# vinhisreal/YOLO-LitePi

Measured on AMD Instinct MI355X. Metric: images/sec end-to-end (det+NMS+clf) 640x640 batch64, higher is better.
Workload: dtype f16; 1 GPU; configs[2]: full det+NMS+ROI+ShuffleNetV2 pipeline, fp16, batch=64/GPU, 640x640, inputs resident in HBM; classifier=ShuffleNetV2 x1.0, 91 classes, seeded random weights, 64x64 ROIs, min_area=50, max_det=300, steps_in_flight=3, distinct_input_batches=4, global_batch=64, boxes_pre_area_filter_rank0=413

## Files before the change

yolo-litepi_amd/csrc/conv_kernels.hip:

```cpp
#include "common.h"
#include "conv.h"
#include "conv_bounds.h"
#include <type_traits>
#include <algorithm>
#include <utility>

namespace lp {

typedef _Float16 half_t;
typedef _Float16 half8 __attribute__((ext_vector_type(8)));
typedef _Float16 half4 __attribute__((ext_vector_type(4)));
typedef _Float16 half2v __attribute__((ext_vector_type(2)));
typedef float floatx4 __attribute__((ext_vector_type(4)));
typedef float floatx2 __attribute__((ext_vector_type(2)));
typedef uint32_t u32x4 __attribute__((ext_vector_type(4)));

enum { EPI_PLAIN = 0, EPI_SHUFFLE = 1 };

#define LP_STAMP(k)                                                                                   \
  if (a.stamps && threadIdx.x == 0)                                                                   \
    a.stamps[((size_t)(blockIdx.z * gridDim.y + blockIdx.y) * gridDim.x + blockIdx.x) * 16 + (k)] = \
        (k) == 0 ? wall_clock64() : clock64();

template <typename T> struct Tr;
// ... 435 lines not shown
  }
  LP_STAMP(10)

  const int oy = oy0 + ly;
  const int oxb = ox0 + wx * 20 + (col & 3);
  if constexpr (T2 > 0) {
    typename Tr<T>::frag w2f[T2][TailSteps<T>::per_nt(NT)];
    floatx4 bias2[T2];
    tail_load<T, NT, T2>(a, lane, g, w2f, bias2);
    ConvArgs a2 = a;
    a2.Cout = a.Cout2; a2.act = a.act2; a2.res = nullptr;
#pragma unroll
    for (int p = 0; p < 5; ++p) {
      const int ox = oxb + p * 4;
      if (oy < a.Hout && ox < a.Wout) {
        const long pix = (n * a.Hout + oy) * a.Wout + ox;
        floatx4 v[NT];
#pragma unroll
        for (int t = 0; t < NT; ++t) v[t] = acc[t][p];
        if (a.act == ACT_SILU) tail_store<T, NT, T2, ACT_SILU>(a2, pix, g, v, bias_r, w2f, bias2);
        else tail_store<T, NT, T2, ACT_NONE>(a2, pix, g, v, bias_r, w2f, bias2);
      }
    }
  } else {
    if (a.act == ACT_SILU) epilogue_tile<T, NT, ACT_SILU>(a, acc, bias_r, n, ns, g, oy, oxb);
    else if (a.act == ACT_RELU) epilogue_tile<T, NT, ACT_RELU>(a, acc, bias_r, n, ns, g, oy, oxb);
    else epilogue_tile<T, NT, ACT_NONE>(a, acc, bias_r, n, ns, g, oy, oxb);
  }
  LP_STAMP(11)
  if (a.stamps && threadIdx.x == 0) a.stamps[((size_t)(blockIdx.z * gridDim.y + blockIdx.y) * gridDim.x + blockIdx.x) * 16 + 12] = wall_clock64();
}


#define BN_STAMP(k)                                                                                                   \
  if (a.stamps && threadIdx.x == 0)                                                                                 \
    a.stamps[((size_t)blockIdx.y * gridDim.x + blockIdx.x) * 16 + (k)] = ((k) == 0 || (k) == 15) ? wall_clock64() : clock64();
template <typename T, int NT, int P1, int P2, bool SEP, int T2 = 0, int SG = 0, bool CL = false>
__global__ __launch_bounds__(256, ((NT >= 4 || P1 >= 15 || (NT == 2 && P1 == 5)) ? 2 : 3)) void bottleneck_mfma_kernel(const BneckArgs a) {
  static_assert(!CL || (SEP && T2 > 0 && SG > 0), "CL: the staged tile must survive conv_a, and cv2's gather must be the straight-line form");
  extern __shared__ __attribute__((aligned(16))) char smem[];
  constexpr int G = Tr<T>::G;
  const int tid = threadIdx.x, lane = tid & 63, wave = tid >> 6;
  const int g = lane >> 4, col = lane & 15;
  const int tile_id = a.tile_major ? blockIdx.x : blockIdx.y;
  const int ty = (int)((tile_id * a.rcp_tx) >> 16), tx = tile_id - ty * a.tiles_x;
  const int n = a.tile_major ? blockIdx.y : blockIdx.x;
  BN_STAMP(0)
  BN_STAMP(1)
  const int TH = a.TH, TW = a.TW, LW = a.LW, PS = a.PS, S = a.steps, CG = a.CG;
  const int PSA = CL ? a.PSA : PS;
  const int CGA = CL ? a.kg : CG;
  const int c1off = CL ? (a.kg - CG) * 16 : 0;
  const int oy0 = ty * TH, ox0 = tx * TW;
  const int IH = TH + 4, IW = TW + 4, H1 = TH + 2, W1 = TW + 2;
  const int R1 = H1 * W1, R2 = TH * TW;
  const int n1 = (R1 + 15) >> 4, n2 = (R2 + 15) >> 4;

  int* lds_toff = reinterpret_cast<int*>(smem);
  const int wbytes = S * NT * 1024;
  const u32x4* lds_w1 = reinterpret_cast<const u32x4*>(smem + 512);
  const u32x4* lds_w2 = reinterpret_cast<const u32x4*>(smem + 512 + wbytes);
  constexpr int SR = TailSteps<T>::per_nt(NT);
  const int w3frags = T2 > 0 ? T2 * (a.sg + SR) : 0;
  const u32x4* lds_w3 = reinterpret_cast<const u32x4*>(smem + 512 + 2 * wbytes);
  char* tile = smem + 512 + 2 * wbytes + w3frags * 1024;
  char* tile2 = SEP ? tile + (TH + 4) * LW * PSA : tile;
  for (int q = tid; q < S * 4; q += 256) {
    int tap = (int)(((unsigned)q * a.rcp_cg) >> 16);
    const int cg = q - tap * CG;
    tap = tap > 8 ? 8 : tap;
    const int ky = (tap * 21846) >> 16, kx = tap - 3 * ky;
    lds_toff[q] = (ky * LW + kx) * PSA + c1off + cg * 16;
    if (CL) lds_toff[64 + q] = (ky * LW + kx) * PS + cg * 16;
  }

  const int RS = LW * (PSA >> 4), PSs = PSA >> 4;
  const int pcs = (RS + 63) >> 6;
  constexpr int NPC = CL ? 4 : 3;
  const int st_pitch = CL ? a.cat_pitch : a.in_pitch;
  const int iy0 = oy0 - 2, ix0 = ox0 - 2;
  const char* zeros = reinterpret_cast<const char*>(a.zeros);
  {
    const int wave_s = __builtin_amdgcn_readfirstlane(wave);
    for (int p = wave_s; p < 2 * S * NT; p += 4) {
      const u32x4* src = p < S * NT ? reinterpret_cast<const u32x4*>(a.w1) + p * 64 : reinterpret_cast<const u32x4*>(a.w2) + (p - S * NT) * 64;
      LP_GLDS16(src + lane, smem + 512 + p * 1024);
    }
    for (int p = wave_s; p < w3frags; p += 4) LP_GLDS16(reinterpret_cast<const u32x4*>(a.w3) + p * 64 + lane, smem + 512 + 2 * wbytes + p * 1024);
    const char* in_b = reinterpret_cast<const char*>(CL ? a.cat : a.in);
// ... 14 lines not shown
        const bool rok = gy >= 0 && gy < a.H;
        const char* rowp = in_b + ((long)(n * a.H + (rok ? gy : 0)) * a.W + ix0) * st_pitch * (long)sizeof(T);
#pragma unroll
        for (int pc = 0; pc < NPC; ++pc) {
          if (pc < pcs) {
            const char* src = (rok && lok[pc]) ? rowp + voff[pc] : zeros;
            if (inrs[pc]) LP_GLDS16(src, tile + (iy * RS + pc * 64) * 16);
          }
        }
      }
    } else {
      const int nitems = IH * pcs;
      for (int it = wave_s; it < nitems; it += 4) {
        const int iy = (int)(((unsigned)it * a.rcp_pcs) >> 16), pc = it - iy * pcs;
        const int gy = iy0 + iy;
        const char* rowp = in_b + ((long)(n * a.H + gy) * a.W + ix0) * st_pitch * (long)sizeof(T);
        const int sl = pc * 64 + lane;
        const int ix = (int)(((unsigned)sl * a.rcp_ps) >> 16), cgs = sl - ix * PSs;
        const int gx = ix0 + ix;
        const bool ok = gy >= 0 && gy < a.H && gx >= 0 && gx < a.W && ix < IW && cgs < CGA;
        const char* src = ok ? rowp + (ix * st_pitch + cgs * G) * (int)sizeof(T) : zeros;
        if (sl < RS) LP_GLDS16(src, tile + (iy * RS + pc * 64) * 16);
      }
    }
  }
  BN_STAMP(2)
  floatx4 bias1[NT], bias2[NT];
#pragma unroll
  for (int t = 0; t < NT; ++t) {
    bias1[t] = *reinterpret_cast<const floatx4*>(a.b1 + g * 4 * NT + t * 4);
    bias2[t] = *reinterpret_cast<const floatx4*>(a.b2 + g * 4 * NT + t * 4);
  }

  int pk1[P1], pb1[P1];
#pragma unroll
  for (int i = 0; i < P1; ++i) {
    int p = (wave + 4 * i) * 16 + col;
    p = p < R1 ? p : R1 - 1;
    const int py = (int)(((unsigned)p * a.rcp_w1) >> 16), px = p - py * W1;
    pk1[i] = (py << 16) | px;
    pb1[i] = (py * LW + px) * PSA;
  }
  floatx4 acc[NT][P1];
#pragma unroll
  for (int t = 0; t < NT; ++t)
#pragma unroll
    for (int i = 0; i < P1; ++i) acc[t][i] = floatx4{0.f, 0.f, 0.f, 0.f};
  asm volatile("s_waitcnt vmcnt(0) lgkmcnt(0)" ::: "memory");
  __builtin_amdgcn_s_barrier();
  BN_STAMP(3)
  for (int s = 0; s < S; ++s) {
    const int toff = lds_toff[4 * s + g];
    typename Tr<T>::frag af[NT], bf[P1];
#pragma unroll
    for (int t = 0; t < NT; ++t) af[t] = as_frag<T>(lds_w1[(s * NT + t) * 64 + lane]);
#pragma unroll
    for (int i = 0; i < P1; ++i) bf[i] = as_frag<T>(*reinterpret_cast<const u32x4*>(tile + pb1[i] + toff));
#pragma unroll
    for (int t = 0; t < NT; ++t)
#pragma unroll
      for (int i = 0; i < P1; ++i) acc[t][i] = Tr<T>::mma(af[t], bf[i], acc[t][i]);
  }
  BN_STAMP(4)
  if (!SEP) {
    asm volatile("s_waitcnt lgkmcnt(0)" ::: "memory");
    __builtin_amdgcn_s_barrier();
  }
  auto write_mid = [&](auto interior_tag) {
    constexpr bool INTERIOR = decltype(interior_tag)::value;
#pragma unroll
    for (int i = 0; i < P1; ++i) {
      const int p = (wave + 4 * i) * 16 + col;
      if (wave + 4 * i < n1 && p < R1) {
        const int py = pk1[i] >> 16, px = pk1[i] & 0xffff;
        bool inside = true;
        if constexpr (!INTERIOR) {
          const int gy = oy0 - 1 + py, gx = ox0 - 1 + px;
          inside = gy >= 0 && gy < a.H && gx >= 0 && gx < a.W;
        }
        T* dst = reinterpret_cast<T*>(tile2 + (py * LW + px) * PS) + g * 4 * NT;
#pragma unroll
        for (int t = 0; t < NT; ++t) {
          if (g * 4 * NT + t * 4 < a.C) {
            typename Tr<T>::quad q;
            const floatx4 y = act4<T, ACT_SILU>(acc[t][i], bias1[t]);
#pragma unroll
            for (int r = 0; r < 4; ++r) q[r] = inside ? (T)y[r] : (T)0.f;
            *reinterpret_cast<typename Tr<T>::quad*>(dst + t * 4) = q;
          }
        }
      }
    }
  };
  if (oy0 >= 1 && ox0 >= 1 && oy0 + TH + 1 <= a.H && ox0 + TW + 1 <= a.W) write_mid(std::true_type{});
  else write_mid(std::false_type{});
  asm volatile("s_waitcnt lgkmcnt(0)" ::: "memory");
  __builtin_amdgcn_s_barrier();

  BN_STAMP(5)
  int pk2[P2], pb2[P2];
#pragma unroll
  for (int i = 0; i < P2; ++i) {
    int p = (wave + 4 * i) * 16 + col;
    p = p < R2 ? p : R2 - 1;
    const int oy = (int)(((unsigned)p * a.rcp_tw) >> 16), ox = p - oy * TW;
    pk2[i] = (oy << 16) | ox;
    pb2[i] = (oy * LW + ox) * PS;
  }
  floatx4 acc2[NT][P2];
#pragma unroll
  for (int t = 0; t < NT; ++t)
#pragma unroll
    for (int i = 0; i < P2; ++i) acc2[t][i] = floatx4{0.f, 0.f, 0.f, 0.f};
  for (int s = 0; s < S; ++s) {
    const int toff = lds_toff[(CL ? 64 : 0) + 4 * s + g];
    typename Tr<T>::frag af[NT], bf[P2];
#pragma unroll
    for (int t = 0; t < NT; ++t) af[t] = as_frag<T>(lds_w2[(s * NT + t) * 64 + lane]);
#pragma unroll
    for (int i = 0; i < P2; ++i) bf[i] = as_frag<T>(*reinterpret_cast<const u32x4*>(tile2 + pb2[i] + toff));
#pragma unroll
    for (int t = 0; t < NT; ++t)
#pragma unroll
      for (int i = 0; i < P2; ++i) acc2[t][i] = Tr<T>::mma(af[t], bf[i], acc2[t][i]);
  }
  BN_STAMP(6)
  const int chbase = g * 4 * NT;
  if constexpr (T2 == 0) {
#pragma unroll
    for (int i = 0; i < P2; ++i) {
      const int p = (wave + 4 * i) * 16 + col;
      const int gy = oy0 + (pk2[i] >> 16), gx = ox0 + (pk2[i] & 0xffff);
      if (wave + 4 * i < n2 && p < R2 && gy < a.H && gx < a.W) {
        const int pix = (n * a.H + gy) * a.W + gx;
        floatx4 v[NT];
#pragma unroll
        for (int t = 0; t < NT; ++t) v[t] = acc2[t][i];
        const T* xres = SEP ? reinterpret_cast<const T*>(tile + (((pk2[i] >> 16) + 2) * LW + (pk2[i] & 0xffff) + 2) * PSA + c1off) + chbase
                            : reinterpret_cast<const T*>(a.in) + eoff(pix, a.in_pitch) + chbase;
        store_lane_at<T, NT, ACT_SILU>(reinterpret_cast<T*>(a.out) + eoff(pix, a.out_pitch) + chbase, xres, chbase, a.C, v, bias2);
      }
    }
  } else {
    constexpr int SGMAX = sizeof(T) == 2 ? 3 : 6;
    const int sg_n = SG > 0 ? SG : a.sg;
    const int ST = sg_n + SR;
    floatx4 bias3[T2];
#pragma unroll
    for (int t = 0; t < T2; ++t) bias3[t] = *reinterpret_cast<const floatx4*>(a.b3 + g * 4 * T2 + t * 4);
    constexpr int LA = P2 < 4 ? P2 : 4;
    auto tile_pixel = [&](int i, bool& valid) {
      const int p = (wave + 4 * i) * 16 + col;
      const int gy = oy0 + (pk2[i] >> 16), gx = ox0 + (pk2[i] & 0xffff);
      valid = wave + 4 * i < n2 && p < R2 && gy < a.H && gx < a.W;
      return valid ? (n * a.H + gy) * a.W + gx : 0;
    };
    constexpr bool FLAT = SG > 0;
    constexpr int SGN = FLAT ? SG : SGMAX;
    typename Tr<T>::quad xq[LA][NT];
    auto request = [&](int i, u32x4 (&dst)[SGN], typename Tr<T>::quad (&xdst)[NT]) {
      bool valid;
      const int pix = tile_pixel(i, valid);
      if (FLAT && !SEP) {
        const T* xp = reinterpret_cast<const T*>(a.in) + eoff(pix, a.in_pitch);
#pragma unroll
        for (int t = 0; t < NT; ++t) xdst[t] = *reinterpret_cast<const typename Tr<T>::quad*>(xp + (chbase + t * 4 < a.C ? chbase + t * 4 : 0));
      }
      const T* catpix = reinterpret_cast<const T*>(a.cat) + eoff(pix, a.cat_pitch);
      const char* ldspix = tile + (((pk2[i] >> 16) + 2) * LW + (pk2[i] & 0xffff) + 2) * PSA;
#pragma unroll
      for (int s = 0; s < SGN; ++s) {
        const int grp = 4 * s + g;
        if constexpr (CL) {
          dst[s] = *reinterpret_cast<const u32x4*>(ldspix + (grp < a.kg ? grp * 16 : 0));
        } else if (FLAT) {
          dst[s] = *reinterpret_cast<const u32x4*>(catpix + (grp < a.kg ? grp * G : 0));
        } else {
          dst[s] = u32x4{0u, 0u, 0u, 0u};
          if (s < a.sg && valid && grp < a.kg) dst[s] = *reinterpret_cast<const u32x4*>(catpix + grp * G);
        }
      }
    };
    u32x4 bgq[LA][SGN];
#pragma unroll
    for (int i = 0; i < LA; ++i) request(i, bgq[i], xq[i]);
    __builtin_amdgcn_sched_barrier(0);
#pragma unroll
    for (int i = 0; i < P2; ++i) {
      if (!FLAT && wave + 4 * i >= n2) continue;
      bool valid;
      const int pix = tile_pixel(i, valid);
      typename Tr<T>::frag bg[SGN];
#pragma unroll
      for (int s = 0; s < SGN; ++s) {
        const unsigned m = (!FLAT || (valid && 4 * s + g < a.kg)) ? 0xffffffffu : 0u;
        bg[s] = as_frag<T>(bgq[i % LA][s] & m);
      }
      typename Tr<T>::quad xqi[NT];
#pragma unroll
      for (int t = 0; t < NT; ++t) xqi[t] = xq[i % LA][t];
      if (i + LA < P2) {
        request(i + LA, bgq[i % LA], xq[i % LA]);
        __builtin_amdgcn_sched_barrier(0);
      }
      const T* xres = SEP ? reinterpret_cast<const T*>(tile + (((pk2[i] >> 16) + 2) * LW + (pk2[i] & 0xffff) + 2) * PSA + c1off) + chbase
                          : reinterpret_cast<const T*>(a.in) + eoff(pix, a.in_pitch) + chbase;
      T yl[NT][4];
#pragma unroll
      for (int t = 0; t < NT; ++t) {
        typename Tr<T>::quad xr;
#pragma unroll
        for (int r = 0; r < 4; ++r) xr[r] = (T)0.f;
        if (SEP) {
          if (chbase + t * 4 < a.C) xr = *reinterpret_cast<const typename Tr<T>::quad*>(xres + t * 4);
        } else if (FLAT) {
          if (valid && chbase + t * 4 < a.C) xr = xqi[t];
        } else if (valid && chbase + t * 4 < a.C) xr = *reinterpret_cast<const typename Tr<T>::quad*>(xres + t * 4);
        const floatx4 y = act4<T, ACT_SILU>(acc2[t][i], bias2[t]);
#pragma unroll
        for (int r = 0; r < 4; ++r) {
          const T q = (T)y[r];
          yl[t][r] = (T)((float)q + (float)xr[r]);
        }
      }
      typename Tr<T>::frag bq[SR];
      if constexpr (sizeof(T) == 2) {
#pragma unroll
        for (int s = 0; s < SR; ++s)
#pragma unroll
          for (int r = 0; r < 4; ++r) {
            bq[s][r] = yl[2 * s][r];
            bq[s][4 + r] = (2 * s + 1 < NT) ? yl[(2 * s + 1 < NT) ? 2 * s + 1 : 0][r] : (T)0.f;
          }
      } else {
#pragma unroll
        for (int s = 0; s < SR; ++s)
#pragma unroll
          for (int r = 0; r < 4; ++r) bq[s][r] = yl[s][r];
      }
      floatx4 o[T2];
#pragma unroll
      for (int t = 0; t < T2; ++t) o[t] = floatx4{0.f, 0.f, 0.f, 0.f};
#pragma unroll
      for (int s = 0; s < SGN; ++s) {
        if (FLAT || s < a.sg) {
#pragma unroll
          for (int t = 0; t < T2; ++t) o[t] = Tr<T>::mma(as_frag<T>(lds_w3[(t * ST + s) * 64 + lane]), bg[s], o[t]);
        }
      }
#pragma unroll
      for (int s = 0; s < SR; ++s)
#pragma unroll
        for (int t = 0; t < T2; ++t) o[t] = Tr<T>::mma(as_frag<T>(lds_w3[(t * ST + sg_n + s) * 64 + lane]), bq[s], o[t]);
      if (valid) {
        T* o3 = reinterpret_cast<T*>(a.out3) + eoff(pix, a.out3_pitch) + g * 4 * T2;
        if (a.act3 == ACT_SILU) store_lane_at<T, T2, ACT_SILU>(o3, nullptr, g * 4 * T2, a.C3, o, bias3);
        else store_lane_at<T, T2, ACT_NONE>(o3, nullptr, g * 4 * T2, a.C3, o, bias3);
      }
    }
  }
  BN_STAMP(7)
  BN_STAMP(15)
}

template <typename T, int NT, int NP, int EPI, bool UPS = false>
__global__ __launch_bounds__(256) void conv1x1_mfma_kernel(const ConvArgs a) {
  extern __shared__ __attribute__((aligned(16))) char smem[];
  constexpr int G = Tr<T>::G;
  const int tid = threadIdx.x;
  const int lane = tid & 63, wave = tid >> 6;
  const int g = lane >> 4, col = lane & 15;
  const int ns = blockIdx.y;
  const int S = a.steps;
  const int CG = a.Cin / G;

  const long M = a.m_dyn ? (long)(*a.m_dyn) * a.pix_per_item : (long)a.M;
  const long ntiles = (M + 64 * NP - 1) / (64 * NP);
  if ((long)blockIdx.x >= ntiles) return;

  u32x4* lds_w = reinterpret_cast<u32x4*>(smem);
  const u32x4* wsrc = reinterpret_cast<const u32x4*>(a.wpk) + (size_t)ns * S * NT * 64;
  for (int i = tid; i < S * NT * 64; i += 256) lds_w[i] = wsrc[i];
  __syncthreads();
  const T* in = reinterpret_cast<const T*>(a.in);
  floatx4 bias_r[NT];
#pragma unroll
  for (int t = 0; t < NT; ++t) bias_r[t] = *reinterpret_cast<const floatx4*>(a.bias + ns * 16 * NT + g * 4 * NT + t * 4);

  for (long tile = blockIdx.x; tile < ntiles; tile += gridDim.x) {
    const long pix0 = (tile * 4 + wave) * 16 * NP;
    if (pix0 >= M) continue;
    const T* src[NP];
// ... 1006 lines not shown
template <typename T> static bool launch_bneck(const BottleneckPair& bp, const BneckArgs& a, dim3 grid, hipStream_t st) {
  return for_each_entry(cplan::kBneckTiles, [&](auto i) {
    constexpr int TILE = (int)decltype(i)::value;
    constexpr cplan::BneckTile t = cplan::kBneckTiles[TILE];
    if (bp.TH != t.th || bp.TW != t.tw) return false;
    if (bp.T2 == 0)
      return for_each_entry(cplan::kBneckNT, [&](auto n) {
        constexpr int nt = cplan::kBneckNT[decltype(n)::value];
        if constexpr (nt <= t.max_nt) {
          if (bp.NT != nt) return false;
          launch_bneck_kernel<T, nt, t.p1, t.p2, 0, 0, false>(a, grid, bp.lds_bytes, st);
          return true;
        } else {
          return false;
        }
      });
    if constexpr (sizeof(T) == 2) {
      static_assert(cplan::kBneckMaxSgF16 == 3, "one launch_bneck_tail line per SG");
      switch (bp.sg) {
        case 1: return launch_bneck_tail<T, TILE, 1>(bp, a, grid, st);
        case 2: return launch_bneck_tail<T, TILE, 2>(bp, a, grid, st);
        case 3: return launch_bneck_tail<T, TILE, 3>(bp, a, grid, st);
        default: return false;
      }
    } else {
      return bp.sg <= cplan::kBneckMaxSgF32 && launch_bneck_tail<T, TILE, 0>(bp, a, grid, st);
    }
  });
}

void BottleneckPair::launch(const View& in, const View& out, int N, hipStream_t st, const View* cat) const {
  LP_CHECK(in.C == C && in.H == out.H && in.W == out.W, LP_ERR_STATE, "bottleneck: view mismatch");
  LP_CHECK((in.pitch % 8) == 0 && (out.pitch % 4) == 0, LP_ERR_STATE, "unaligned channel pitch");
  LP_CHECK(span_ok(N, in) && span_ok(N, out) && (!cat || span_ok(N, *cat)), LP_ERR_ARG, "bottleneck: a tensor of batch %d exceeds 2^31 elements", N);
  BneckArgs k;
  memset(&k, 0, sizeof(k));
  k.in = in.base; k.out = out.base; k.w1 = a.d_w.p; k.w2 = b.d_w.p; k.b1 = a.d_bias.as<float>(); k.b2 = b.d_bias.as<float>();
  k.zeros = a.d_bias.as<float>() + round_up(C, 64);
  k.N = N; k.H = in.H; k.W = in.W; k.C = C; k.in_pitch = in.pitch; k.out_pitch = out.pitch;
  k.TH = TH; k.TW = TW; k.tiles_x = ceil_div(in.W, TW); k.LW = LW; k.PS = PS; k.CG = CG; k.steps = steps;
  if (T2) {
    LP_CHECK(cat && cat->base && cat->H == in.H && cat->W == in.W && out.C >= C3, LP_ERR_STATE, "bottleneck+cv2: concat view missing or output too narrow");
    k.w3 = d_w3.p; k.b3 = d_b3.as<float>(); k.cat = cat->base; k.cat_pitch = cat->pitch;
    k.out3 = out.base; k.out3_pitch = out.pitch; k.C3 = C3; k.act3 = act3; k.kg = kg; k.sg = sg;
    k.out = nullptr;
    if (cl) {
      const size_t es = prec == LP_FP16 ? 2 : 4;
      LP_CHECK(reinterpret_cast<const char*>(in.base) == reinterpret_cast<const char*>(cat->base) + (size_t)(kg * cplan::group(prec) - C) * es &&
                   in.pitch == cat->pitch,
               LP_ERR_STATE, "bottleneck %s: planned with the input as the concat's last stored segment, launched with another view", name.c_str());
      k.PSA = PSA;
    }
  } else {
    LP_CHECK(out.C >= C, LP_ERR_STATE, "bottleneck: output view too narrow");
  }
  const int tiles_y = ceil_div(in.H, TH);
  k.rcp_tx = rcp16_checked(k.tiles_x, k.tiles_x * tiles_y);
  k.rcp_cg = rcp_cg; k.rcp_ps = rcp_ps; k.rcp_pcs = rcp_pcs; k.rcp_w1 = rcp_w1; k.rcp_tw = rcp_tw;
  k.tile_major = tile_major_order();
  dim3 grid(N, k.tiles_x * tiles_y);
  if (k.tile_major) grid = dim3(k.tiles_x * tiles_y, N);
  static const char* stamp_path = getenv("LITEPI_BNECK_STAMPS");
  DevBuf d_stamps;
  if (stamp_path && *stamp_path) {
    d_stamps.alloc((size_t)grid.x * grid.y * 16 * 8);
    LP_HIP(hipMemsetAsync(d_stamps.p, 0, (size_t)grid.x * grid.y * 16 * 8, st));
    k.stamps = d_stamps.as<unsigned long long>();
// ... 144 lines not shown
```

yolo-litepi_amd/csrc/conv_plan.h:

```cpp
#pragma once
#include <cstddef>

#include "../../include/litepi.h"

namespace lp {
namespace cplan {

constexpr int cdiv(int a, int b) { return (a + b - 1) / b; }
inline int group(int prec) { return prec == LP_FP16 ? 8 : 4; }

inline unsigned rcp16(int d, int range) {
  const unsigned m = (65536u + d - 1) / d;
  for (int x = 0; x < range; ++x)
    if ((int)((x * m) >> 16) != x / d) return 0;
  return m;
}

struct Variant { int nt, t2; };
constexpr Variant kConv3x3[] = {{1, 0}, {2, 0}, {3, 0}, {4, 0}, {4, 4}, {2, 1}};
constexpr Variant kConvS2[] = {{1, 0}, {2, 0}, {3, 0}, {4, 0}, {1, 1}, {2, 2}, {4, 4}};
constexpr int s2_unroll(int steps) { return steps >= 5 ? 4 : 1; }
constexpr int kConv1x1[] = {1, 2, 3, 4};
constexpr int kStemCO[] = {8, 16, 32};
struct BneckTile { int th, tw, p1, p2, max_nt; bool tail, cl; };
// ... 123 lines not shown
    p.CK = cin;
    p.CGc = cin / G;
    p.nchunks = 1;
    p.steps = cdiv(p.CGc, 4);
    while (p.NT > 1 && (size_t)p.steps * p.NT * 1024 > 96 * 1024) --p.NT;
    p.nsplits = cdiv(tiles_total, p.NT);
    p.lds_bytes = (size_t)p.steps * p.NT * 1024;
    if (p.lds_bytes > 160 * 1024) p.plan_err = "conv1x1 weights do not fit LDS";
  }
  return p;
}

inline bool conv_tail_supported(int k, int stride, int cmid, int cout2) {
  if (k != 3 || cmid % 8 != 0) return false;
  const int nt = cdiv(cmid, 16), t2 = cdiv(cout2, 16);
  return t2 > 0 && (stride == 1 ? has_variant(kConv3x3, nt, t2) : stride == 2 ? has_variant(kConvS2, nt, t2) : false);
}
inline int tail_steps(int prec, int nt) { return prec == LP_FP16 ? (nt + 1) / 2 : nt; }

struct BneckTail {
  int cat_global = 0, c3 = 0;
  bool in_is_last_stored = false;
  bool cl = false;
};
struct BneckTiling {
  bool ok = false;
  int TH = 8, TW = 40, LW = 0;
  size_t lds_bytes = 0;
  int T2 = 0, kg = 0, sg = 0;
  bool cl = false;
  int PSA = 0;
};

inline BneckTiling plan_bneck(int prec, int c, int h, int w, int batch_hint, const BneckTail* tail) {
  BneckTiling p;
  const int G = group(prec);
  if (c % 8 != 0 || c > 64) return p;
  const int nt = cdiv(c, 16), cg = c / G;
  size_t extra_lds = 0;
  if (tail) {
    if (tail->cat_global <= 0 || tail->cat_global % G != 0 || tail->c3 % 8 != 0) return p;
    p.T2 = cdiv(tail->c3, 16);
    p.kg = tail->cat_global / G;
    p.sg = cdiv(p.kg, 4);
    if (!has_variant(kBneckTails, nt, p.T2) || p.sg > (prec == LP_FP16 ? kBneckMaxSgF16 : kBneckMaxSgF32)) return p;
    extra_lds = (size_t)p.T2 * (p.sg + tail_steps(prec, nt)) * 1024;
  }
  const int steps = cdiv(9 * cg, 4);
  if (steps * 4 > 128) return p;
  const int pss = lds_pixel_slots(cg);
  const int B = batch_hint > 0 ? batch_hint : 1;
  const bool sep = nt == 1;
  const int kg_cl = (tail && tail->in_is_last_stored) ? p.kg : 0;
  const bool try_cl = tail && tail->cl && kg_cl > cg && kg_cl <= 4 && prec == LP_FP16 && nt == 1;
  for (int pass = try_cl ? 0 : 1; pass < 2; ++pass) {
    const bool clp = pass == 0;
    const int pssa = clp ? (kg_cl | 1) : pss;
    long best = -1;
    for (const BneckTile& t : kBneckTiles) {
      const int TH = t.th, TW = t.tw;
      if (nt > t.max_nt || (tail && !t.tail) || (clp && !t.cl)) continue;
      if ((TH == 20 || TH == 10) && (long)cdiv(h, TH) * cdiv(w, TW) * B > 512) continue;
      int l = TW + 4;
      if (cg <= 1) while (l % 16 != 2) ++l;
      if (cdiv(l * pssa, 64) > (clp ? 4 : 8)) continue;
      const size_t need = 512 + (size_t)2 * steps * nt * 1024 + extra_lds + (size_t)(TH + 4) * l * pssa * 16 + (size_t)(sep ? TH + 2 : 0) * l * pss * 16;
// ... 21 lines not shown
```

yolo-litepi_amd/csrc/detector_plan.cpp:

```cpp
#include "detector.h"
#include <cstring>

#include <algorithm>
#include <optional>
#include <set>

namespace lp {

struct PlanSwitches {
  static bool on(const char* name) { return getenv(name) != nullptr; }
  bool no_c2f = on("LITEPI_NO_C2F");
  bool c2f_bb80 = on("LITEPI_C2F_BB80");
  std::string c2f_skip = getenv("LITEPI_C2F_SKIP") ? std::string(";") + getenv("LITEPI_C2F_SKIP") + ";" : std::string();
  int c2f_min_batch = getenv("LITEPI_C2F_MIN_BATCH") ? atoi(getenv("LITEPI_C2F_MIN_BATCH")) : 4;
  bool c2f_store_all = on("LITEPI_C2F_STORE_ALL");
  bool c2f_xcv1 = on("LITEPI_C2F_XCV1");
  bool no_c2f_xcv1 = on("LITEPI_NO_C2F_XCV1");
  bool no_s2c = on("LITEPI_NO_S2C");
  bool no_s2lds = on("LITEPI_NO_S2LDS");
  bool no_s2tail = on("LITEPI_NO_S2TAIL");
  bool no_sppf_fused = on("LITEPI_NO_SPPF_FUSED");
  bool no_sibling = on("LITEPI_NO_SIBLING");
  bool no_bneck = on("LITEPI_NO_BNECK");
  bool no_cv2fuse = on("LITEPI_NO_CV2FUSE");
// ... 826 lines not shown
  tensors_.push_back(M);
  op.in = tin; op.out = (int)tensors_.size() - 1;
  ops_.push_back(op);
  done[sib] = 1;
  return true;
}

bool Planner::try_bottleneck(const ConvSite& c) {
  const int i = c.i, tin = c.tin, tout = c.tout, Cin = c.Cin, Cout = c.Cout;
  const NcnnLayer& l = L[i];
  if (sw.no_bneck || c.res >= 0 || c.k != 3 || c.s != 1 || Cin != Cout || tin == input_tensor || impl_ != IMPL_MFMA ||
      fused_act[i] != ACT_SILU || tensors_[tout].segs.size() != 1 || tensors_[tin].segs.size() != 1)
    return false;
  const int j = sole_consumer(tout);
  if (j < 0 || L[j].type != "Convolution" || is_tail(j) || done[j]) return false;
  const NcnnLayer& lb = L[j];
  const int tb = cinfo[j].tout;
  const int jadd = sole_consumer(tb);
  if (lb.ipar(1, 1) != 3 || lb.ipar(3, 1) != 1 || lb.ipar(0) != Cout || lb.in_ch != Cout || fused_act[j] != ACT_SILU || jadd < 0 ||
      L[jadd].type != "BinaryOp" || is_tail(jadd))
    return false;
  const NcnnLayer& add = L[jadd];
  const int ta = get(add.inputs[0]), tb2 = get(add.inputs[1]);
  const int other = ta == tb ? tb2 : ta;
  const int tfinal = get(add.outputs[0]);
  const Tensor& TI = tensors_[tin];
  if (other != tin || TI.Cp != tensors_[tfinal].Cp || TI.Cp != tensors_[tout].Cp || !BottleneckPair::supported(prec_, impl_, TI.Cp, TI.H, TI.W, maxB_))
    return false;
  std::optional<Cv2Match> f = match_bneck_cv2(tin, tfinal);
  if (f) { f->cv2.w = &f->w; f->cv2.bias = &f->b; }
  const int jc = f ? f->conv : -1, tcat = f ? f->t_cat : -1;
  const int tdst = jc >= 0 ? cinfo[jc].tout : tfinal;
  ensure_buffer(tdst);
  std::vector<float> wa, ba, wb, bb;
  repack(l, TI, tensors_[tout], 0, tensors_[tout].Cp, wa, ba);
  repack(lb, tensors_[tout], tensors_[tfinal], 0, tensors_[tfinal].Cp, wb, bb);
  d.bnecks_.emplace_back(new BottleneckPair());
  d.bnecks_.back()->name = l.name + "+" + lb.name + (jc >= 0 ? "+" + L[jc].name : std::string());
  d.bnecks_.back()->build(prec_, TI.Cp, wa, ba, wb, bb, TI.H, TI.W, maxB_, jc >= 0 ? &f->cv2 : nullptr);
  double macs = 2.0 * 9.0 * Cin * Cout * TI.H * TI.W;
  if (jc >= 0) macs += (double)L[jc].in_ch * L[jc].ipar(0) * TI.H * TI.W;
  macs_ += macs;
  DetOp op;
  op.kind = DetOp::BNECK; op.layer = d.bnecks_.back()->name; op.conv = (int)d.bnecks_.size() - 1;
  op.flops = 2.0 * macs;
  op.bytes = 2.0 * TI.C * TI.H * TI.W * esd + (double)(l.weight.size() + lb.weight.size()) * esd;
  if (jc >= 0)
    op.bytes = ((double)(tensors_[tcat].C - TI.C) + TI.C + tensors_[tdst].C) * TI.H * TI.W * esd +
               (double)(l.weight.size() + lb.weight.size() + L[jc].weight.size()) * esd;
  op.in = tin; op.out = tdst; op.in2 = tcat;
  ops_.push_back(op);
  if (jc >= 0) done[jc] = 1;
  done[j] = 1; done[jadd] = 1;
  return true;
}

std::optional<Planner::Cv2Match> Planner::match_bneck_cv2(int tin, int tfinal) {
  const int cc = sole_consumer(tfinal);
  if (sw.no_cv2fuse || cc < 0 || L[cc].type != "Concat" || canon(L[cc].inputs.back()) != tensors_[tfinal].name) return std::nullopt;
  const int tO = get(L[cc].outputs[0]);
  const int j3 = sole_consumer(tO);
  if (!zero_copy_concat(cc) || j3 < 0 || L[j3].type != "Convolution" || is_tail(j3) || done[j3] || L[j3].ipar(1, 1) != 1 ||
      L[j3].ipar(3, 1) != 1 || fuse_up.count(j3) || tensors_[tfinal].buf != tensors_[tO].buf || tensors_[tO].parent >= 0)
    return std::nullopt;
  const int t3 = cinfo[j3].tout;
  const Tensor &TI = tensors_[tin], &TO = tensors_[tO];
// ... 443 lines not shown
```

Baseline: 130,600 images/sec.

## Strength-reduce bottleneck kernel pixel indexing and predicate masks to cut VGPRs

Replaces per-pixel divide-based coordinate recomputation in the fused bottleneck kernel with an incremental tile walker that carries LDS and global byte offsets in registers, using scalar deltas and 24-bit multiplies. Validity and channel checks become precomputed bitmasks applied with AND instead of branches, and interior/edge paths are specialized for the second stage and tail. Raises the occupancy hint to 4 for one fp16 variant and adds a 2^31-byte span guard so 32-bit byte offsets are safe. The aim is to reduce VALU address math and register pressure; the risks are heavier code specialization and the changed occupancy hint causing spills.

```diff
diff --git a/yolo-litepi_amd/csrc/conv_kernels.hip b/yolo-litepi_amd/csrc/conv_kernels.hip
--- a/yolo-litepi_amd/csrc/conv_kernels.hip
+++ b/yolo-litepi_amd/csrc/conv_kernels.hip
@@ -491,11 +491,27 @@
 }
 
 
-#define BN_STAMP(k)                                                                                                   \
+struct TileWalk {
+  int x, y;
+  __device__ __forceinline__ bool next(int RW, int q64, int r64) {
+    x += r64;
+    const bool wrap = x >= RW;
+    x -= wrap ? RW : 0;
+    y += q64 + (wrap ? 1 : 0);
+    return wrap;
+  }
+};
+__device__ __forceinline__ half4 and_mask(half4 q, unsigned m) {
+  typedef unsigned u32x2_t __attribute__((ext_vector_type(2)));
+  return __builtin_bit_cast(half4, __builtin_bit_cast(u32x2_t, q) & m);
+}
+__device__ __forceinline__ floatx4 and_mask(floatx4 q, unsigned m) { return __builtin_bit_cast(floatx4, __builtin_bit_cast(u32x4, q) & m); }
+#define BN_STAMP(k)                                                                                                 \
   if (a.stamps && threadIdx.x == 0)                                                                                 \
     a.stamps[((size_t)blockIdx.y * gridDim.x + blockIdx.x) * 16 + (k)] = ((k) == 0 || (k) == 15) ? wall_clock64() : clock64();
 template <typename T, int NT, int P1, int P2, bool SEP, int T2 = 0, int SG = 0, bool CL = false>
-__global__ __launch_bounds__(256, ((NT >= 4 || P1 >= 15 || (NT == 2 && P1 == 5)) ? 2 : 3)) void bottleneck_mfma_kernel(const BneckArgs a) {
+__global__ __launch_bounds__(256, ((NT >= 4 || P1 >= 15 || (NT == 2 && P1 == 5)) ? 2 : (sizeof(T) == 2 && NT == 1 && P1 == 12 && T2 == 1 && SG == 1) ? 4 : 3))
+void bottleneck_mfma_kernel(const BneckArgs a) {
   static_assert(!CL || (SEP && T2 > 0 && SG > 0), "CL: the staged tile must survive conv_a, and cv2's gather must be the straight-line form");
   extern __shared__ __attribute__((aligned(16))) char smem[];
   constexpr int G = Tr<T>::G;
@@ -513,7 +529,7 @@
   const int oy0 = ty * TH, ox0 = tx * TW;
   const int IH = TH + 4, IW = TW + 4, H1 = TH + 2, W1 = TW + 2;
   const int R1 = H1 * W1, R2 = TH * TW;
-  const int n1 = (R1 + 15) >> 4, n2 = (R2 + 15) >> 4;
+  const int n2 = (R2 + 15) >> 4;
 
   int* lds_toff = reinterpret_cast<int*>(smem);
   const int wbytes = S * NT * 1024;
@@ -594,14 +610,53 @@
     bias2[t] = *reinterpret_cast<const floatx4*>(a.b2 + g * 4 * NT + t * 4);
   }
 
-  int pk1[P1], pb1[P1];
-#pragma unroll
-  for (int i = 0; i < P1; ++i) {
-    int p = (wave + 4 * i) * 16 + col;
-    p = p < R1 ? p : R1 - 1;
-    const int py = (int)(((unsigned)p * a.rcp_w1) >> 16), px = p - py * W1;
-    pk1[i] = (py << 16) | px;
-    pb1[i] = (py * LW + px) * PSA;
+  constexpr bool CH_WHOLE = NT <= 2;
+  const int chbase = g * 4 * NT;
+  const bool chok = chbase < a.C;
+  const int c_lim = CH_WHOLE ? 0x7fffffff : a.C;
+  int xsel[NT];
+  unsigned chm[NT];
+#pragma unroll
+  for (int t = 0; t < NT; ++t) {
+    const bool qok = CH_WHOLE ? chok : chbase + t * 4 < a.C;
+    xsel[t] = qok ? chbase + t * 4 : 0;
+    chm[t] = qok ? 0xffffffffu : 0u;
+  }
+
+  const bool interior1 = oy0 >= 1 && ox0 >= 1 && oy0 + TH + 1 <= a.H && ox0 + TW + 1 <= a.W;
+  const int p0 = wave * 16 + col;
+  const bool last1 = p0 + 64 * (P1 - 1) < R1;
+  int pb1[P1];
+  int pm1[CL ? P1 : 1];
+  unsigned in1 = 0xffffffffu;
+  {
+    const int q64 = (int)((64u * a.rcp_w1) >> 16), r64 = 64 - q64 * W1;
+    const int lrow = q64 * LW + r64;
+    int dP = lrow * PSA, dPw = dP + (LW - W1) * PSA, dM = lrow * PS, dMw = dM + (LW - W1) * PS;
+    asm("" : "+s"(dP), "+s"(dPw), "+s"(dM), "+s"(dMw));
+    TileWalk w;
+    w.y = (int)(__umul24(p0, a.rcp_w1) >> 16);
+    w.x = p0 - (int)__umul24(w.y, W1);
+    const int lp0 = (int)__umul24(w.y, LW) + w.x;
+    int pb = (int)__umul24(lp0, PSA), pm = (int)__umul24(lp0, PS);
+#pragma unroll
+    for (int i = 0; i < P1; ++i) {
+      if (i > 0) {
+        const bool wrap = w.next(W1, q64, r64);
+        pb += wrap ? dPw : dP;
+        if (CL) pm += wrap ? dMw : dM;
+      }
+      if (i == P1 - 1) {
+        pb = last1 ? pb : ((H1 - 1) * LW + W1 - 1) * PSA;
+        pm = last1 ? pm : ((H1 - 1) * LW + W1 - 1) * PS;
+      }
+      if (!interior1) {
+        const bool inside = (unsigned)(w.y + oy0 - 1) < (unsigned)a.H && (unsigned)(w.x + ox0 - 1) < (unsigned)a.W;
+        in1 &= inside ? 0xffffffffu : ~(1u << i);
+      }
+      pb1[i] = pb;
+      if (CL) pm1[i] = pm;
+    }
   }
   floatx4 acc[NT][P1];
 #pragma unroll
@@ -632,43 +687,79 @@
     constexpr bool INTERIOR = decltype(interior_tag)::value;
 #pragma unroll
     for (int i = 0; i < P1; ++i) {
-      const int p = (wave + 4 * i) * 16 + col;
-      if (wave + 4 * i < n1 && p < R1) {
-        const int py = pk1[i] >> 16, px = pk1[i] & 0xffff;
-        bool inside = true;
-        if constexpr (!INTERIOR) {
-          const int gy = oy0 - 1 + py, gx = ox0 - 1 + px;
-          inside = gy >= 0 && gy < a.H && gx >= 0 && gx < a.W;
-        }
-        T* dst = reinterpret_cast<T*>(tile2 + (py * LW + px) * PS) + g * 4 * NT;
-#pragma unroll
-        for (int t = 0; t < NT; ++t) {
-          if (g * 4 * NT + t * 4 < a.C) {
-            typename Tr<T>::quad q;
-            const floatx4 y = act4<T, ACT_SILU>(acc[t][i], bias1[t]);
-#pragma unroll
-            for (int r = 0; r < 4; ++r) q[r] = inside ? (T)y[r] : (T)0.f;
-            *reinterpret_cast<typename Tr<T>::quad*>(dst + t * 4) = q;
-          }
-        }
-      }
+      if (i == P1 - 1 && !last1) continue;
+      T* dst = reinterpret_cast<T*>(tile2 + (CL ? pm1[CL ? i : 0] : pb1[i])) + chbase;
+      const unsigned inside = INTERIOR ? 0xffffffffu : 0u - ((in1 >> i) & 1u);
+#pragma unroll
+      for (int t = 0; t < NT; ++t) {
+        if (CH_WHOLE || chbase + t * 4 < a.C) {
+          typename Tr<T>::quad q;
+          const floatx4 y = act4<T, ACT_SILU>(acc[t][i], bias1[t]);
+#pragma unroll
+          for (int r = 0; r < 4; ++r) q[r] = (T)y[r];
+          if constexpr (!INTERIOR) q = and_mask(q, inside);
+          *reinterpret_cast<typename Tr<T>::quad*>(dst + t * 4) = q;
+        }
+      }
+      __builtin_amdgcn_sched_barrier(0);
     }
   };
-  if (oy0 >= 1 && ox0 >= 1 && oy0 + TH + 1 <= a.H && ox0 + TW + 1 <= a.W) write_mid(std::true_type{});
-  else write_mid(std::false_type{});
+  if (!CH_WHOLE || chok) {
+    if (interior1) write_mid(std::true_type{});
+    else write_mid(std::false_type{});
+  }
   asm volatile("s_waitcnt lgkmcnt(0)" ::: "memory");
   __builtin_amdgcn_s_barrier();
 
   BN_STAMP(5)
-  int pk2[P2], pb2[P2];
-#pragma unroll
-  for (int i = 0; i < P2; ++i) {
-    int p = (wave + 4 * i) * 16 + col;
-    p = p < R2 ? p : R2 - 1;
-    const int oy = (int)(((unsigned)p * a.rcp_tw) >> 16), ox = p - oy * TW;
-    pk2[i] = (oy << 16) | ox;
-    pb2[i] = (oy * LW + ox) * PS;
-  }
+  const bool interior2 = oy0 + TH <= a.H && ox0 + TW <= a.W;
+  const bool last2 = p0 + 64 * (P2 - 1) < R2;
+  const int xsh = (2 * LW + 2) * PS;
+  int pb2[P2];
+  int pa2[CL ? P2 : 1];
+  unsigned gp2[P2];
+  unsigned ok2 = 0xffffffffu;
+  const int out_pitch_b = (T2 > 0 ? a.out3_pitch : a.out_pitch) * (int)sizeof(T), cat_pitch_b = a.cat_pitch * (int)sizeof(T), in_pitch_b = a.in_pitch * (int)sizeof(T);
+  auto walk2 = [&](auto interior_tag) {
+    constexpr bool INTERIOR = decltype(interior_tag)::value;
+    const int q64 = (int)((64u * a.rcp_tw) >> 16), r64 = 64 - q64 * TW;
+    const int lrow = q64 * LW + r64, grow = q64 * a.W + r64;
+    int dP = lrow * PS, dPw = dP + (LW - TW) * PS, dA = lrow * PSA, dAw = dA + (LW - TW) * PSA;
+    unsigned dG = grow, dGw = grow + a.W - TW;
+    asm("" : "+s"(dP), "+s"(dPw), "+s"(dA), "+s"(dAw), "+s"(dG), "+s"(dGw));
+    const int hlim = a.H - oy0, wlim = a.W - ox0;
+    TileWalk w;
+    w.y = (int)(__umul24(p0, a.rcp_tw) >> 16);
+    w.x = p0 - (int)__umul24(w.y, TW);
+    int pb = (int)__umul24(__umul24(w.y, LW) + w.x, PS);
+    int pa = (int)__umul24(__umul24(w.y + 2, LW) + w.x + 2, PSA);
+    unsigned gp = __umul24(w.y, a.W) + w.x;
+#pragma unroll
+    for (int i = 0; i < P2; ++i) {
+      if (i > 0) {
+        const bool wrap = w.next(TW, q64, r64);
+        pb += wrap ? dPw : dP;
+        gp += wrap ? dGw : dG;
+        if (CL) pa += wrap ? dAw : dA;
+      }
+      unsigned gpl = gp;
+      if (i == P2 - 1 || !INTERIOR) {
+        bool ok = i == P2 - 1 ? last2 : true;
+        if (i == P2 - 1) {
+          pb = ok ? pb : ((TH - 1) * LW + TW - 1) * PS;
+          pa = ok ? pa : ((TH + 1) * LW + TW + 1) * PSA;
+        }
+        if (!INTERIOR) ok = ok && w.y < hlim && w.x < wlim;
+        gpl = ok ? gp : 0u;
+        ok2 &= ok ? 0xffffffffu : ~(1u << i);
+      }
+      pb2[i] = pb;
+      gp2[i] = gpl;
+      if constexpr (CL) pa2[i] = pa;
+    }
+  };
+  if (interior2) walk2(std::true_type{});
+  else walk2(std::false_type{});
   floatx4 acc2[NT][P2];
 #pragma unroll
   for (int t = 0; t < NT; ++t)
@@ -687,21 +778,27 @@
       for (int i = 0; i < P2; ++i) acc2[t][i] = Tr<T>::mma(af[t], bf[i], acc2[t][i]);
   }
   BN_STAMP(6)
-  const int chbase = g * 4 * NT;
+  const size_t pix0 = (size_t)((n * a.H + oy0) * a.W + ox0);
+  const char* in0 = reinterpret_cast<const char*>(a.in) + pix0 * a.in_pitch * sizeof(T);
+  char* out0 = reinterpret_cast<char*>(T2 > 0 ? a.out3 : a.out) + pix0 * (size_t)out_pitch_b;
   if constexpr (T2 == 0) {
-#pragma unroll
-    for (int i = 0; i < P2; ++i) {
-      const int p = (wave + 4 * i) * 16 + col;
-      const int gy = oy0 + (pk2[i] >> 16), gx = ox0 + (pk2[i] & 0xffff);
-      if (wave + 4 * i < n2 && p < R2 && gy < a.H && gx < a.W) {
-        const int pix = (n * a.H + gy) * a.W + gx;
+    auto plain = [&](auto interior_tag) {
+      constexpr bool INTERIOR = decltype(interior_tag)::value;
+#pragma unroll
+      for (int i = 0; i < P2; ++i) {
+        if ((i == P2 - 1 || !INTERIOR) && !((ok2 >> i) & 1u)) continue;
         floatx4 v[NT];
 #pragma unroll
         for (int t = 0; t < NT; ++t) v[t] = acc2[t][i];
-        const T* xres = SEP ? reinterpret_cast<const T*>(tile + (((pk2[i] >> 16) + 2) * LW + (pk2[i] & 0xffff) + 2) * PSA + c1off) + chbase
-                            : reinterpret_cast<const T*>(a.in) + eoff(pix, a.in_pitch) + chbase;
-        store_lane_at<T, NT, ACT_SILU>(reinterpret_cast<T*>(a.out) + eoff(pix, a.out_pitch) + chbase, xres, chbase, a.C, v, bias2);
-      }
+        const T* xres = SEP ? reinterpret_cast<const T*>(tile + pb2[i] + xsh) + chbase
+                            : reinterpret_cast<const T*>(in0 + __umul24(gp2[i], in_pitch_b)) + chbase;
+        store_lane_at<T, NT, ACT_SILU>(reinterpret_cast<T*>(out0 + __umul24(gp2[i], out_pitch_b)) + chbase, xres, chbase, c_lim, v, bias2);
+        __builtin_amdgcn_sched_barrier(0);
+      }
+    };
+    if (!CH_WHOLE || chok) {
+      if (interior2) plain(std::true_type{});
+      else plain(std::false_type{});
     }
   } else {
     constexpr int SGMAX = sizeof(T) == 2 ? 3 : 6;
@@ -711,115 +808,125 @@
 #pragma unroll
     for (int t = 0; t < T2; ++t) bias3[t] = *reinterpret_cast<const floatx4*>(a.b3 + g * 4 * T2 + t * 4);
     constexpr int LA = P2 < 4 ? P2 : 4;
-    auto tile_pixel = [&](int i, bool& valid) {
-      const int p = (wave + 4 * i) * 16 + col;
-      const int gy = oy0 + (pk2[i] >> 16), gx = ox0 + (pk2[i] & 0xffff);
-      valid = wave + 4 * i < n2 && p < R2 && gy < a.H && gx < a.W;
-      return valid ? (n * a.H + gy) * a.W + gx : 0;
-    };
     constexpr bool FLAT = SG > 0;
     constexpr int SGN = FLAT ? SG : SGMAX;
-    typename Tr<T>::quad xq[LA][NT];
-    auto request = [&](int i, u32x4 (&dst)[SGN], typename Tr<T>::quad (&xdst)[NT]) {
-      bool valid;
-      const int pix = tile_pixel(i, valid);
-      if (FLAT && !SEP) {
-        const T* xp = reinterpret_cast<const T*>(a.in) + eoff(pix, a.in_pitch);
-#pragma unroll
-        for (int t = 0; t < NT; ++t) xdst[t] = *reinterpret_cast<const typename Tr<T>::quad*>(xp + (chbase + t * 4 < a.C ? chbase + t * 4 : 0));
-      }
-      const T* catpix = reinterpret_cast<const T*>(a.cat) + eoff(pix, a.cat_pitch);
-      const char* ldspix = tile + (((pk2[i] >> 16) + 2) * LW + (pk2[i] & 0xffff) + 2) * PSA;
-#pragma unroll
-      for (int s = 0; s < SGN; ++s) {
-        const int grp = 4 * s + g;
-        if constexpr (CL) {
-          dst[s] = *reinterpret_cast<const u32x4*>(ldspix + (grp < a.kg ? grp * 16 : 0));
-        } else if (FLAT) {
-          dst[s] = *reinterpret_cast<const u32x4*>(catpix + (grp < a.kg ? grp * G : 0));
+    unsigned gsel[FLAT ? SGN : 1], gmask[FLAT ? SGN : 1];
+#pragma unroll
+    for (int s = 0; s < (FLAT ? SGN : 0); ++s) {
+      const int grp = 4 * s + g;
+      gsel[s] = grp < a.kg ? grp * 16 : 0;
+      gmask[s] = grp < a.kg ? 0xffffffffu : 0u;
+    }
+    const char* cat0 = reinterpret_cast<const char*>(a.cat) + pix0 * a.cat_pitch * sizeof(T);
+    const bool ch3ok = T2 > 2 || g * 4 * T2 < a.C3;
+    const int c3_lim = T2 <= 2 ? 0x7fffffff : a.C3;
+    auto tail = [&](auto interior_tag) {
+      constexpr bool INTERIOR = decltype(interior_tag)::value;
+      auto tile_ok = [&](int i) { return (i < P2 - 1 && INTERIOR) || ((ok2 >> i) & 1u) != 0; };
+      typename Tr<T>::quad xq[LA][NT];
+      auto request = [&](int i, u32x4 (&dst)[SGN], typename Tr<T>::quad (&xdst)[NT]) {
+        if (FLAT && !SEP) {
+          const T* xp = reinterpret_cast<const T*>(in0 + __umul24(gp2[i], in_pitch_b));
+#pragma unroll
+          for (int t = 0; t < NT; ++t) xdst[t] = *reinterpret_cast<const typename Tr<T>::quad*>(xp + xsel[t]);
+        }
+        const char* catpix = cat0 + __umul24(gp2[i], cat_pitch_b);
+        const char* ldspix = CL ? tile + pa2[CL ? i : 0] : tile;
+#pragma unroll
+        for (int s = 0; s < SGN; ++s) {
+          if constexpr (CL) {
+            dst[s] = *reinterpret_cast<const u32x4*>(ldspix + gsel[s]);
+          } else if constexpr (FLAT) {
+            dst[s] = *reinterpret_cast<const u32x4*>(catpix + gsel[s]);
+          } else {
+            dst[s] = u32x4{0u, 0u, 0u, 0u};
+            if (s < a.sg && tile_ok(i) && 4 * s + g < a.kg) dst[s] = *reinterpret_cast<const u32x4*>(catpix + (4 * s + g) * 16);
+          }
+        }
+      };
+      u32x4 bgq[LA][SGN];
+#pragma unroll
+      for (int i = 0; i < LA; ++i) request(i, bgq[i], xq[i]);
+      __builtin_amdgcn_sched_barrier(0);
+#pragma unroll
+      for (int i = 0; i < P2; ++i) {
+        if (!FLAT && wave + 4 * i >= n2) continue;
+        const bool valid = tile_ok(i);
+        const unsigned vmask = (i < P2 - 1 && INTERIOR) ? 0xffffffffu : (valid ? 0xffffffffu : 0u);
+        typename Tr<T>::frag bg[SGN];
+#pragma unroll
+        for (int s = 0; s < SGN; ++s) {
+          if constexpr (FLAT) bg[s] = as_frag<T>(bgq[i % LA][s] & (gmask[s] & vmask));
+          else bg[s] = as_frag<T>(bgq[i % LA][s]);
+        }
+        typename Tr<T>::quad xqi[NT];
+#pragma unroll
+        for (int t = 0; t < NT; ++t) xqi[t] = xq[i % LA][t];
+        if (i + LA < P2) {
+          request(i + LA, bgq[i % LA], xq[i % LA]);
+          __builtin_amdgcn_sched_barrier(0);
+        }
+        T yl[NT][4];
+#pragma unroll
+        for (int t = 0; t < NT; ++t) {
+          typename Tr<T>::quad xr;
+#pragma unroll
+          for (int r = 0; r < 4; ++r) xr[r] = (T)0.f;
+          if (SEP) {
+            const char* xpix = CL ? tile + pa2[CL ? i : 0] + c1off : tile + pb2[i] + xsh;
+            xr = and_mask(*reinterpret_cast<const typename Tr<T>::quad*>(reinterpret_cast<const T*>(xpix) + xsel[t]), chm[t]);
+          } else if (FLAT) {
+            xr = and_mask(xqi[t], chm[t] & vmask);
+          } else if (valid && chm[t]) {
+            xr = *reinterpret_cast<const typename Tr<T>::quad*>(reinterpret_cast<const T*>(in0 + __umul24(gp2[i], in_pitch_b)) + chbase + t * 4);
+          }
+          const floatx4 y = act4<T, ACT_SILU>(acc2[t][i], bias2[t]);
+#pragma unroll
+          for (int r = 0; r < 4; ++r) {
+            const T q = (T)y[r];
+            yl[t][r] = (T)((float)q + (float)xr[r]);
+          }
+        }
+        typename Tr<T>::frag bq[SR];
+        if constexpr (sizeof(T) == 2) {
+#pragma unroll
+          for (int s = 0; s < SR; ++s)
+#pragma unroll
+            for (int r = 0; r < 4; ++r) {
+              bq[s][r] = yl[2 * s][r];
+              bq[s][4 + r] = (2 * s + 1 < NT) ? yl[(2 * s + 1 < NT) ? 2 * s + 1 : 0][r] : (T)0.f;
+            }
         } else {
-          dst[s] = u32x4{0u, 0u, 0u, 0u};
-          if (s < a.sg && valid && grp < a.kg) dst[s] = *reinterpret_cast<const u32x4*>(catpix + grp * G);
-        }
+#pragma unroll
+          for (int s = 0; s < SR; ++s)
+#pragma unroll
+            for (int r = 0; r < 4; ++r) bq[s][r] = yl[s][r];
+        }
+        floatx4 o[T2];
+#pragma unroll
+        for (int t = 0; t < T2; ++t) o[t] = floatx4{0.f, 0.f, 0.f, 0.f};
+#pragma unroll
+        for (int s = 0; s < SGN; ++s) {
+          if (FLAT || s < a.sg) {
+#pragma unroll
+            for (int t = 0; t < T2; ++t) o[t] = Tr<T>::mma(as_frag<T>(lds_w3[(t * ST + s) * 64 + lane]), bg[s], o[t]);
+          }
+        }
+#pragma unroll
+        for (int s = 0; s < SR; ++s)
+#pragma unroll
+          for (int t = 0; t < T2; ++t) o[t] = Tr<T>::mma(as_frag<T>(lds_w3[(t * ST + sg_n + s) * 64 + lane]), bq[s], o[t]);
+        if (valid && ch3ok) {
+          T* o3 = reinterpret_cast<T*>(out0 + __umul24(gp2[i], out_pitch_b)) + g * 4 * T2;
+          if (a.act3 == ACT_SILU) store_lane_at<T, T2, ACT_SILU>(o3, nullptr, g * 4 * T2, c3_lim, o, bias3);
+          else store_lane_at<T, T2, ACT_NONE>(o3, nullptr, g * 4 * T2, c3_lim, o, bias3);
+        }
+        __builtin_amdgcn_sched_barrier(0);
+        asm volatile("" ::: "memory");
       }
     };
-    u32x4 bgq[LA][SGN];
-#pragma unroll
-    for (int i = 0; i < LA; ++i) request(i, bgq[i], xq[i]);
-    __builtin_amdgcn_sched_barrier(0);
-#pragma unroll
-    for (int i = 0; i < P2; ++i) {
-      if (!FLAT && wave + 4 * i >= n2) continue;
-      bool valid;
-      const int pix = tile_pixel(i, valid);
-      typename Tr<T>::frag bg[SGN];
-#pragma unroll
-      for (int s = 0; s < SGN; ++s) {
-        const unsigned m = (!FLAT || (valid && 4 * s + g < a.kg)) ? 0xffffffffu : 0u;
-        bg[s] = as_frag<T>(bgq[i % LA][s] & m);
-      }
-      typename Tr<T>::quad xqi[NT];
-#pragma unroll
-      for (int t = 0; t < NT; ++t) xqi[t] = xq[i % LA][t];
-      if (i + LA < P2) {
-        request(i + LA, bgq[i % LA], xq[i % LA]);
-        __builtin_amdgcn_sched_barrier(0);
-      }
-      const T* xres = SEP ? reinterpret_cast<const T*>(tile + (((pk2[i] >> 16) + 2) * LW + (pk2[i] & 0xffff) + 2) * PSA + c1off) + chbase
-                          : reinterpret_cast<const T*>(a.in) + eoff(pix, a.in_pitch) + chbase;
-      T yl[NT][4];
-#pragma unroll
-      for (int t = 0; t < NT; ++t) {
-        typename Tr<T>::quad xr;
-#pragma unroll
-        for (int r = 0; r < 4; ++r) xr[r] = (T)0.f;
-        if (SEP) {
-          if (chbase + t * 4 < a.C) xr = *reinterpret_cast<const typename Tr<T>::quad*>(xres + t * 4);
-        } else if (FLAT) {
-          if (valid && chbase + t * 4 < a.C) xr = xqi[t];
-        } else if (valid && chbase + t * 4 < a.C) xr = *reinterpret_cast<const typename Tr<T>::quad*>(xres + t * 4);
-        const floatx4 y = act4<T, ACT_SILU>(acc2[t][i], bias2[t]);
-#pragma unroll
-        for (int r = 0; r < 4; ++r) {
-          const T q = (T)y[r];
-          yl[t][r] = (T)((float)q + (float)xr[r]);
-        }
-      }
-      typename Tr<T>::frag bq[SR];
-      if constexpr (sizeof(T) == 2) {
-#pragma unroll
-        for (int s = 0; s < SR; ++s)
-#pragma unroll
-          for (int r = 0; r < 4; ++r) {
-            bq[s][r] = yl[2 * s][r];
-            bq[s][4 + r] = (2 * s + 1 < NT) ? yl[(2 * s + 1 < NT) ? 2 * s + 1 : 0][r] : (T)0.f;
-          }
-      } else {
-#pragma unroll
-        for (int s = 0; s < SR; ++s)
-#pragma unroll
-          for (int r = 0; r < 4; ++r) bq[s][r] = yl[s][r];
-      }
-      floatx4 o[T2];
-#pragma unroll
-      for (int t = 0; t < T2; ++t) o[t] = floatx4{0.f, 0.f, 0.f, 0.f};
-#pragma unroll
-      for (int s = 0; s < SGN; ++s) {
-        if (FLAT || s < a.sg) {
-#pragma unroll
-          for (int t = 0; t < T2; ++t) o[t] = Tr<T>::mma(as_frag<T>(lds_w3[(t * ST + s) * 64 + lane]), bg[s], o[t]);
-        }
-      }
-#pragma unroll
-      for (int s = 0; s < SR; ++s)
-#pragma unroll
-        for (int t = 0; t < T2; ++t) o[t] = Tr<T>::mma(as_frag<T>(lds_w3[(t * ST + sg_n + s) * 64 + lane]), bq[s], o[t]);
-      if (valid) {
-        T* o3 = reinterpret_cast<T*>(a.out3) + eoff(pix, a.out3_pitch) + g * 4 * T2;
-        if (a.act3 == ACT_SILU) store_lane_at<T, T2, ACT_SILU>(o3, nullptr, g * 4 * T2, a.C3, o, bias3);
-        else store_lane_at<T, T2, ACT_NONE>(o3, nullptr, g * 4 * T2, a.C3, o, bias3);
-      }
-    }
+    if (interior2) tail(std::true_type{});
+    else tail(std::false_type{});
   }
   BN_STAMP(7)
   BN_STAMP(15)
@@ -1892,7 +1999,9 @@
 void BottleneckPair::launch(const View& in, const View& out, int N, hipStream_t st, const View* cat) const {
   LP_CHECK(in.C == C && in.H == out.H && in.W == out.W, LP_ERR_STATE, "bottleneck: view mismatch");
   LP_CHECK((in.pitch % 8) == 0 && (out.pitch % 4) == 0, LP_ERR_STATE, "unaligned channel pitch");
-  LP_CHECK(span_ok(N, in) && span_ok(N, out) && (!cat || span_ok(N, *cat)), LP_ERR_ARG, "bottleneck: a tensor of batch %d exceeds 2^31 elements", N);
+  const int es = prec == LP_FP16 ? 2 : 4;
+  auto bytes_ok = [&](const View& v) { return !v.base || cplan::bneck_span_ok(N, v.H, v.W, v.pitch, es); };
+  LP_CHECK(bytes_ok(in) && bytes_ok(out) && (!cat || bytes_ok(*cat)), LP_ERR_ARG, "bottleneck: a tensor of batch %d exceeds 2^31 bytes", N);
   BneckArgs k;
   memset(&k, 0, sizeof(k));
   k.in = in.base; k.out = out.base; k.w1 = a.d_w.p; k.w2 = b.d_w.p; k.b1 = a.d_bias.as<float>(); k.b2 = b.d_bias.as<float>();
diff --git a/yolo-litepi_amd/csrc/conv_plan.h b/yolo-litepi_amd/csrc/conv_plan.h
--- a/yolo-litepi_amd/csrc/conv_plan.h
+++ b/yolo-litepi_amd/csrc/conv_plan.h
@@ -179,6 +179,10 @@
   int PSA = 0;
 };
 
+inline bool bneck_span_ok(long n, long h, long w, long pitch, int elem_bytes) {
+  return (double)n * (double)h * (double)w * (double)pitch * elem_bytes < 2147483648.0;
+}
+
 inline BneckTiling plan_bneck(int prec, int c, int h, int w, int batch_hint, const BneckTail* tail) {
   BneckTiling p;
   const int G = group(prec);
diff --git a/yolo-litepi_amd/csrc/detector_plan.cpp b/yolo-litepi_amd/csrc/detector_plan.cpp
--- a/yolo-litepi_amd/csrc/detector_plan.cpp
+++ b/yolo-litepi_amd/csrc/detector_plan.cpp
@@ -882,6 +882,13 @@
   const int jc = f ? f->conv : -1, tcat = f ? f->t_cat : -1;
   const int tdst = jc >= 0 ? cinfo[jc].tout : tfinal;
   ensure_buffer(tdst);
+  auto span_ok = [&](int t) {
+    if (t < 0) return true;
+    const Tensor& X = tensors_[t];
+    const int bi = X.parent >= 0 ? tensors_[X.parent].buf : X.buf;
+    return bi < 0 || cplan::bneck_span_ok(maxB_, X.H, X.W, buffers_[bi].Cp, (int)esd);
+  };
+  if (!span_ok(tin) || !span_ok(tdst) || !span_ok(tcat)) return false;
   std::vector<float> wa, ba, wb, bb;
   repack(l, TI, tensors_[tout], 0, tensors_[tout].Cp, wa, ba);
   repack(lb, tensors_[tout], tensors_[tfinal], 0, tensors_[tfinal].Cp, wb, bb);
```

New measurement: 133,700 images/sec, median of 6. 1.02x the previous value.
